# rfahd1525/Block-Blast-AI---Reinforcement-Learning-Agent

Measured on NVIDIA B200. Metric: env_steps_per_sec, higher is better.
Workload: dtype u64

## Files before the change

block-blast-ai---reinforcement-learning-agent_b200/csrc/bb_env_kernels.cu:

```cuda
#include <cuda_runtime.h>
#include "bb_rules.cuh"
#include "bb_kernels.h"

__device__ BBTables g_bb_tables = {BB_PIECE_ROWS};

__device__ __forceinline__ void bb_load_state(const BBEnvArrays& E, int64_t i, BBState& s) {
    const uint4 a = E.s0[i], b = E.s1[i], c = E.s2[i];
    s.board = (uint64_t)a.x | ((uint64_t)a.y << 32);
    s.pieces = a.z;
    s.aux = a.w;
    s.score = (int32_t)b.x; s.streak = (int32_t)b.y; s.moves = (int32_t)b.z; s.lines_total = (int32_t)b.w;
    s.max_streak = (int32_t)c.x; s.blocks_total = (int32_t)c.y; s.draw_ctr = c.z; s.policy_ctr = c.w;
}

__device__ __forceinline__ void bb_store_state(const BBEnvArrays& E, int64_t i, const BBState& s) {
    E.s0[i] = make_uint4((uint32_t)s.board, (uint32_t)(s.board >> 32), s.pieces, s.aux);
    E.s1[i] = make_uint4((uint32_t)s.score, (uint32_t)s.streak, (uint32_t)s.moves, (uint32_t)s.lines_total);
    E.s2[i] = make_uint4((uint32_t)s.max_streak, (uint32_t)s.blocks_total, s.draw_ctr, s.policy_ctr);
}

__device__ __forceinline__ uint64_t bb_shfl64(uint64_t v, int src) {
    const uint32_t lo = __shfl_sync(0xffffffffu, (uint32_t)v, src);
    const uint32_t hi = __shfl_sync(0xffffffffu, (uint32_t)(v >> 32), src);
    return (uint64_t)lo | ((uint64_t)hi << 32);
}

#ifdef BB_PROFILE
struct BBProf { long long cls = 0, team = 0, rounds = 0, iters = 0, t0 = 0, c0 = 0, c1 = 0, q0 = 0, q1 = 0, units = 0, units_all = 0, unit_cyc = 0; };
__device__ unsigned long long g_pf_units = 0, g_pf_units_max = 0, g_pf_open_cyc = 0, g_pf_unit_cyc = 0, g_pf_H = 0;
#define BB_PF(...) __VA_ARGS__
#else
struct BBProf {};
#define BB_PF(...)
#endif

__device__ __forceinline__ bool bb_warp_solve(bool hard, const BBItem& item, uint32_t trio, const BBTables* T,
                                              BBProf& pf) {
    const unsigned FULL = 0xffffffffu;
    const int lane = threadIdx.x & 31;
    bool solved = false;
    uint32_t next = 0;
    const uint32_t nbr = BB_PLAN_NA(item.plan) + BB_PLAN_NB(item.plan);
    unsigned hmask = __ballot_sync(FULL, hard);
    while (hmask) {
        BB_PF(pf.rounds += 1;)
        const int rem = hard ? (int)(nbr - next) : 0;
        int excl = 32;
        int owner = lane, o_excl = 0, o_rem = 0;
        bool in_team = false;
        int run = 0;
        for (unsigned m = hmask; m && run < 32; m &= m - 1u) {
            const int h = __ffs((int)m) - 1;
            const int r = __shfl_sync(FULL, rem, h);
            if (lane == h) excl = run;
            if (lane >= run && lane < run + r) { owner = h; o_excl = run; o_rem = r; in_team = true; }
            run += r;
        }
        const int served_o = min(o_rem, 32 - o_excl);
        const unsigned team_mask = in_team ? ((served_o >= 32 ? FULL : ((1u << served_o) - 1u)) << o_excl) : 0u;
        BBItem it;
        it.b = bb_shfl64(item.b, owner);
        it.v[0] = bb_shfl64(item.v[0], owner);
        it.v[1] = bb_shfl64(item.v[1], owner);
        it.v[2] = bb_shfl64(item.v[2], owner);
        it.plan = __shfl_sync(FULL, item.plan, owner);
        const uint32_t tr = __shfl_sync(FULL, trio, owner);
        const uint32_t t = __shfl_sync(FULL, next, owner) + (uint32_t)(lane - o_excl);
        BBBranch br;
        br.bb = 0; br.m0 = 0; br.m1 = 0; br.always = 0;
        br.A.pm = br.A.inb = br.A.offs = 0; br.A.meta = 0;
        br.B = br.A;
        BB_PF(pf.q0 = clock64();)
        if (in_team) bb_branch_open(br, it, T, tr, t);
        BB_PF(pf.q1 = clock64(); pf.units = 0;)
        unsigned found = 0;
        for (;;) {
            const bool work = in_team && !(found & team_mask) && ((br.m0 | br.m1) != 0ull);
            if (!__any_sync(FULL, work)) break;
            bool f = false;
            if (work) f = bb_branch_unit(br);
            found |= __ballot_sync(FULL, f);
            BB_PF(pf.units += 1;)
        }
        BB_PF(if (lane == 0) {
            pf.units_all += pf.units; pf.unit_cyc += clock64() - pf.q1;
            atomicAdd(&g_pf_units, (unsigned long long)pf.units);
            atomicMax(&g_pf_units_max, (unsigned long long)pf.units);
            atomicAdd(&g_pf_open_cyc, (unsigned long long)(pf.q1 - pf.q0));
            atomicAdd(&g_pf_unit_cyc, (unsigned long long)(clock64() - pf.q1));
            atomicAdd(&g_pf_H, (unsigned long long)__popc(hmask));
        })
        if (hard) {
            const int served = max(0, min(rem, 32 - excl));
            const unsigned tm = served > 0 ? ((served >= 32 ? FULL : ((1u << served) - 1u)) << excl) : 0u;
            next += (uint32_t)served;
            if (found & tm) { hard = false; solved = true; }
            else if (next >= nbr) hard = false;
        }
        hmask = __ballot_sync(FULL, hard);
    }
    return solved;
}

template <class Src>
__device__ __forceinline__ uint32_t bb_warp_deal(bool pending, uint64_t board, const BBTables* T,
                                                 const Src& src, uint64_t env_id, uint32_t& pieces,
                                                 uint32_t& draw_ctr, BBProf& pf) {
    const unsigned FULL = 0xffffffffu;
    const int lane = threadIdx.x & 31;
    uint32_t attempts = 0;
    unsigned pmask = __ballot_sync(FULL, pending);
    while (pmask) {
        BB_PF(pf.c0 = clock64(); pf.iters += 1;)
        const int P = __popc(pmask);
        const int w = 32 / P;
        const int g = lane / w, r = lane - g * w;
        const bool in_grp = g < P;
        const int owner = in_grp ? bb_select((uint64_t)pmask, g) : lane;
        const unsigned grp_bits = (w == 32 ? FULL : ((1u << w) - 1u));
        const int shift = (in_grp ? g : 0) * w;
        const uint64_t ob = bb_shfl64(board, owner);
        const uint64_t oid = bb_shfl64(env_id, owner);
        const uint32_t octr = __shfl_sync(FULL, draw_ctr, owner);
        const uint32_t oatt = __shfl_sync(FULL, attempts, owner);
        const bool cand = in_grp && (oatt + (uint32_t)r < 100u);
        BBItem item;
        item.b = ob; item.v[0] = item.v[1] = item.v[2] = 0; item.plan = 0;
        uint32_t trio = 0;
        int cls = BB_REJECT;
        if (cand) {
            trio = bb_candidate(src, oid, octr + (uint32_t)r);
            cls = bb_classify(ob, bb_piece(T, trio & 0xFFu), bb_piece(T, (trio >> 8) & 0xFFu),
                              bb_piece(T, (trio >> 16) & 0xFFu), &item);
        }
        const unsigned amask = __ballot_sync(FULL, cls == BB_ACCEPT);
        const unsigned ga = (amask >> shift) & grp_bits;
        const int first_acc = ga ? (__ffs((int)ga) - 1) : w;
        const bool hard = cand && cls == BB_HARD && r < first_acc;
        BB_PF(pf.c1 = clock64(); pf.cls += pf.c1 - pf.c0;)
        const bool solved = bb_warp_solve(hard, item, trio, T, pf);
        BB_PF(pf.team += clock64() - pf.c1;)
        const unsigned okmask = __ballot_sync(FULL, cand && (cls == BB_ACCEPT || solved));
        const unsigned go = (okmask >> shift) & grp_bits;
        const int nvalid = (int)min((uint32_t)w, 100u - oatt);
        const int take = go ? __ffs((int)go) : nvalid;
        const bool done = go != 0u || (oatt + (uint32_t)take >= 100u);
        const uint32_t chosen = __shfl_sync(FULL, trio, (in_grp ? g * w : 0) + take - 1);
        const int my_base = pending ? __popc(pmask & ((1u << lane) - 1u)) * w : 0;
        const int t_take = __shfl_sync(FULL, take, my_base);
        const int t_done = __shfl_sync(FULL, (int)done, my_base);
        const uint32_t t_trio = __shfl_sync(FULL, chosen, my_base);
        if (pending) {
            draw_ctr += (uint32_t)t_take;
            attempts += (uint32_t)t_take;
            pieces = t_trio;
            pending = !t_done;
        }
        pmask = __ballot_sync(FULL, pending);
    }
    return attempts;
}

template <bool RANDOM, bool INJECT>
__global__ void __launch_bounds__(BB_STEP_THREADS, BB_STEP_MIN_BLOCKS)
bb_step_kernel(BBEnvArrays E, BBRewardCfg cfg, const int32_t* __restrict__ actions, int n_steps, int per_step,
               int32_t* __restrict__ actions_out, float* __restrict__ rewards,
               uint8_t* __restrict__ terminated, uint64_t* __restrict__ mask_out,
               int32_t* __restrict__ ep_score, int32_t* __restrict__ ep_len,
               uint32_t* __restrict__ info_out, unsigned long long* __restrict__ stats,
               uint64_t* __restrict__ board_out, uint32_t* __restrict__ pieces_out,
               const uint64_t* __restrict__ mask_in) {
    const BBTables& T = g_bb_tables;
    const int64_t i = (int64_t)blockIdx.x * blockDim.x + threadIdx.x;
    const bool live = i < E.n;
    unsigned st_eps = 0, st_score = 0, st_len = 0, st_max = 0;
    BBTrioSrc src(E.seed);
    if (INJECT) { src.trios = E.trios; src.len = E.trio_len; src.base = E.trio_base; }
    BBState s;
    BBStepOut o;
    int action = 0;
    const uint64_t env_id = (uint64_t)(E.env_offset + (live ? i : 0));
    if (live) {
        bb_load_state(E, i, s);
        if (RANDOM) {
            if (mask_in) {
                const int64_t ms = E.out_stride ? E.out_stride : E.n;
                o.mask[0] = mask_in[i]; o.mask[1] = mask_in[ms + i]; o.mask[2] = mask_in[2 * ms + i];
            } else {
                bb_action_mask(s, &T, o.mask);
            }
        } else {
            action = actions[i];
        }
    } else {
        s.board = 0; s.pieces = 0; s.aux = 0; s.draw_ctr = 0; s.policy_ctr = 0;
        s.score = s.streak = s.moves = s.lines_total = s.max_streak = s.blocks_total = 0;
        o.mask[0] = o.mask[1] = o.mask[2] = 0;
    }
    const int steps = RANDOM ? n_steps : 1;
    BBProf pf;
    BB_PF(pf.t0 = clock64();)
    for (int step = 0; step < steps; ++step) {
        BBMove mv;
        mv.ok = false; mv.needs_deal = false; mv.n = 0; mv.lines = 0; mv.gain = 0;
        if (live) {
            if (RANDOM) {
                const BBPhilox4 r = bb_philox((uint32_t)env_id, (uint32_t)(env_id >> 32), s.policy_ctr,
                                              BB_STREAM_POLICY, (uint32_t)E.seed, (uint32_t)(E.seed >> 32));
                s.policy_ctr += 1;
                action = bb_pick_action(o.mask, r.x);
            }
            mv = bb_env_pre(s, action, &T, o);
        }
        const uint32_t draws = bb_warp_deal(live && mv.ok && mv.needs_deal, s.board, &T, src, env_id,
                                            s.pieces, s.draw_ctr, pf);
        if (live && mv.ok) {
            bb_env_post(s, mv, draws, &T, cfg, src, env_id, E.flags, o, E.ep_end ? E.ep_end + i : nullptr);
            if (o.terminated) {
                st_eps += 1u; st_score += (unsigned)o.ep_score; st_len += (unsigned)o.ep_len;
                st_max = max(st_max, (unsigned)o.ep_score);
            }
        }
        if (RANDOM && per_step && live) {
            const int64_t base = (int64_t)step * E.n + i;
            if (actions_out) actions_out[base] = action;
            if (rewards) rewards[base] = o.reward;
            if (terminated) terminated[base] = (uint8_t)o.terminated;
            if (mask_out) {
                const int64_t mb = (int64_t)step * 3 * E.n + i;
                mask_out[mb] = o.mask[0];
                mask_out[mb + E.n] = o.mask[1];
                mask_out[mb + 2 * E.n] = o.mask[2];
            }
        }
    }
    if (RANDOM && per_step) {
        if (live) bb_store_state(E, i, s);
        actions_out = nullptr; rewards = nullptr; terminated = nullptr; mask_out = nullptr;
    }
    if (live) {
        if (!(RANDOM && per_step)) bb_store_state(E, i, s);
        if (RANDOM && actions_out) actions_out[i] = action;
        if (rewards) rewards[i] = o.reward;
        if (terminated) terminated[i] = (uint8_t)o.terminated;
        if (mask_out) {
            const int64_t ms = E.out_stride ? E.out_stride : E.n;
            mask_out[i] = o.mask[0];
            mask_out[ms + i] = o.mask[1];
            mask_out[2 * ms + i] = o.mask[2];
        }
        if (o.terminated) {
            if (ep_score) ep_score[i] = o.ep_score;
            if (ep_len) ep_len[i] = o.ep_len;
        }
        if (info_out) info_out[i] = o.info;
        if (board_out) board_out[i] = s.board;
        if (pieces_out) pieces_out[i] = s.pieces;
    }
    if (stats) {
        const unsigned FULLM = 0xffffffffu;
        const unsigned long long w_eps = __reduce_add_sync(FULLM, st_eps);
        const unsigned long long w_score = (unsigned long long)__reduce_add_sync(FULLM, st_score & 0xFFFFu) +
                                           ((unsigned long long)__reduce_add_sync(FULLM, st_score >> 16) << 16);
        const unsigned long long w_len = (unsigned long long)__reduce_add_sync(FULLM, st_len & 0xFFFFu) +
                                         ((unsigned long long)__reduce_add_sync(FULLM, st_len >> 16) << 16);
        const unsigned w_max = __reduce_max_sync(FULLM, st_max);
        const unsigned long long nlive = __popc(__ballot_sync(0xffffffffu, live));
        if ((threadIdx.x & 31) == 0) {
            BB_PF(const unsigned long long tot = (unsigned long long)(clock64() - pf.t0);
                  atomicAdd(&stats[4], tot);
                  atomicAdd(&stats[5], (unsigned long long)pf.cls);
                  atomicAdd(&stats[6], (unsigned long long)pf.team);
                  atomicAdd(&stats[7], (unsigned long long)pf.rounds);
                  atomicAdd(&stats[8], (unsigned long long)pf.iters);
                  atomicMax(&stats[9], tot);
                  atomicMax(&stats[10], (unsigned long long)pf.rounds);
                  atomicMax(&stats[63 - (tot & 7)], (tot << 32) | (((unsigned long long)pf.unit_cyc >> 6) << 16) |
                                                        ((unsigned long long)(pf.units_all > 255 ? 255 : pf.units_all) << 8) | (unsigned long long)(pf.rounds > 255 ? 255 : pf.rounds));
                  stats[11] = g_pf_units; stats[12] = g_pf_units_max; stats[13] = g_pf_open_cyc;
                  stats[14] = g_pf_unit_cyc; stats[15] = g_pf_H;
                  atomicAdd(&stats[16 + (tot >> 13 > 31 ? 31 : tot >> 13)], 1ull);
                  atomicAdd(&stats[48 + (pf.rounds > 7 ? 7 : pf.rounds)], 1ull);)
            atomicAdd(&stats[0], nlive * (unsigned long long)n_steps);
            if (w_eps) {
                atomicAdd(&stats[1], w_eps);
                atomicAdd(&stats[2], w_score);
                atomicAdd(&stats[3], w_len);
#ifndef BB_PROFILE
                atomicMax(&stats[4], (unsigned long long)w_max);
#endif
            }
        }
    }
}

__global__ void __launch_bounds__(BB_STEP_THREADS)
bb_reset_kernel(BBEnvArrays E, const uint8_t* __restrict__ reset_mask, uint64_t* __restrict__ mask_out) {
    const BBTables& T = g_bb_tables;
    const int64_t i = (int64_t)blockIdx.x * blockDim.x + threadIdx.x;
    if (i >= E.n) return;
    BBState s;
    bb_load_state(E, i, s);
    if (!reset_mask || reset_mask[i]) {
        BBTrioSrc src(E.seed);
        src.trios = E.trios; src.len = E.trio_len; src.base = E.trio_base;
        bb_reset_state(s, src, (uint64_t)(E.env_offset + i), E.flags);
        bb_store_state(E, i, s);
    }
    if (mask_out) {
        uint64_t m[3];
        bb_action_mask(s, &T, m);
        mask_out[i] = m[0];
        mask_out[E.n + i] = m[1];
        mask_out[2 * E.n + i] = m[2];
    }
}

__global__ void __launch_bounds__(BB_STEP_THREADS)
bb_observe_kernel(BBEnvArrays E, uint64_t* __restrict__ board_out, uint32_t* __restrict__ pieces_out,
                  uint64_t* __restrict__ mask_out) {
    const BBTables& T = g_bb_tables;
    const int64_t i = (int64_t)blockIdx.x * blockDim.x + threadIdx.x;
    if (i >= E.n) return;
    BBState s;
    bb_load_state(E, i, s);
    if (board_out) board_out[i] = s.board;
    if (pieces_out) pieces_out[i] = s.pieces;
    if (mask_out) {
        uint64_t m[3];
        bb_action_mask(s, &T, m);
        mask_out[i] = m[0];
        mask_out[E.n + i] = m[1];
        mask_out[2 * E.n + i] = m[2];
    }
}

#define BB_STREAM_SAMPLE_VALID 3u
__global__ void __launch_bounds__(BB_STEP_THREADS)
bb_sample_valid_kernel(BBEnvArrays E, uint64_t call_counter, int32_t* __restrict__ actions_out) {
    const BBTables& T = g_bb_tables;
    const int64_t i = (int64_t)blockIdx.x * blockDim.x + threadIdx.x;
    if (i >= E.n) return;
    BBState s;
    bb_load_state(E, i, s);
    uint64_t m[3];
    bb_action_mask(s, &T, m);
    const uint64_t env_id = (uint64_t)(E.env_offset + i);
    const BBPhilox4 r = bb_philox((uint32_t)env_id, (uint32_t)(env_id >> 32), (uint32_t)call_counter,
                                  BB_STREAM_SAMPLE_VALID, (uint32_t)E.seed, (uint32_t)(E.seed >> 32));
    actions_out[i] = bb_pick_action(m, r.x);
}

__device__ __forceinline__ int64_t bb_warp_incl_scan(int64_t v) {
    const int lane = threadIdx.x & 31;
#pragma unroll
    for (int o = 1; o < 32; o <<= 1) {
        const int64_t u = __shfl_up_sync(0xffffffffu, v, o);
        if (lane >= o) v += u;
    }
    return v;
}

__device__ __forceinline__ int64_t bb_block_incl_scan(int64_t v, int64_t* total) {
    __shared__ int64_t warp_sums[BB_STEP_THREADS / 32];
    const int lane = threadIdx.x & 31, w = threadIdx.x >> 5;
    v = bb_warp_incl_scan(v);
    if (lane == 31) warp_sums[w] = v;
    __syncthreads();
    if (w == 0) {
        int64_t t = lane < BB_STEP_THREADS / 32 ? warp_sums[lane] : 0;
        t = bb_warp_incl_scan(t);
        if (lane < BB_STEP_THREADS / 32) warp_sums[lane] = t;
    }
// ... 194 lines not shown
```

block-blast-ai---reinforcement-learning-agent_b200/csrc/bb_rules.cuh:

```cuda
#pragma once
#include <stdint.h>

#if defined(__CUDACC__)
#define BB_HD __host__ __device__ __forceinline__
#else
#define BB_HD inline
#endif

#include "bb_piece_table.inc"

#define BB_TABLE_N (BB_NUM_PIECES + 3)
struct alignas(16) BBTableRow {
    uint64_t mask;
    uint64_t inb;
    uint64_t offs;
    uint32_t meta;
    uint32_t pad;
};
struct BBTables { BBTableRow row[BB_TABLE_N]; };

#define BB_META_N(m) ((m) & 0xFu)
#define BB_META_MAXROW(m) (((m) >> 12) & 0xFu)
#define BB_META_MAXCOL(m) (((m) >> 16) & 0xFu)

static const uint64_t BB_HOST_PIECE_MASKS[BB_NUM_PIECES] = BB_PIECE_MASKS;
static const uint64_t BB_HOST_PIECE_INB[BB_NUM_PIECES] = BB_PIECE_INB;
static const uint64_t BB_HOST_PIECE_OFFS[BB_NUM_PIECES] = BB_PIECE_OFFS;
static const uint32_t BB_HOST_PIECE_META[BB_NUM_PIECES] = BB_PIECE_META;

inline void bb_fill_tables(BBTables* t) {
    for (int i = 0; i < BB_TABLE_N; ++i) {
        t->row[i].mask = i < BB_NUM_PIECES ? BB_HOST_PIECE_MASKS[i] : 0;
        t->row[i].inb = i < BB_NUM_PIECES ? BB_HOST_PIECE_INB[i] : 0;
        t->row[i].offs = i < BB_NUM_PIECES ? BB_HOST_PIECE_OFFS[i] : 0;
        t->row[i].meta = i < BB_NUM_PIECES ? BB_HOST_PIECE_META[i] : 0;
        t->row[i].pad = 0;
    }
}

struct BBPiece { uint64_t pm, inb, offs; uint32_t meta; };

BB_HD BBPiece bb_piece(const BBTables* T, uint32_t id) {
    BBPiece p;
#if defined(__CUDA_ARCH__)
    const uint4* r = reinterpret_cast<const uint4*>(&T->row[id]);
    const uint4 a = r[0], b = r[1];
    p.pm = (uint64_t)a.x | ((uint64_t)a.y << 32);
    p.inb = (uint64_t)a.z | ((uint64_t)a.w << 32);
    p.offs = (uint64_t)b.x | ((uint64_t)b.y << 32);
    p.meta = b.z;
#else
    p.pm = T->row[id].mask; p.inb = T->row[id].inb; p.offs = T->row[id].offs; p.meta = T->row[id].meta;
#endif
    return p;
}

BB_HD int bb_popc(uint64_t x) {
#if defined(__CUDA_ARCH__)
    return __popcll(x);
#else
    return __builtin_popcountll(x);
#endif
}
BB_HD int bb_popc32(uint32_t x) {
#if defined(__CUDA_ARCH__)
    return __popc(x);
#else
    return __builtin_popcount(x);
#endif
}
BB_HD int bb_ctz(uint64_t x) {
#if defined(__CUDA_ARCH__)
    const uint32_t lo = (uint32_t)x;
    return lo ? (__ffs((int)lo) - 1) : (31 + __ffs((int)(uint32_t)(x >> 32)));
#else
    return __builtin_ctzll(x);
#endif
}
BB_HD uint32_t bb_mulhi(uint32_t a, uint32_t b) {
#if defined(__CUDA_ARCH__)
    return __umulhi(a, b);
#else
    return (uint32_t)(((uint64_t)a * b) >> 32);
#endif
}
BB_HD int bb_select(uint64_t w, int k) {
#if defined(__CUDA_ARCH__)
    uint32_t x = (uint32_t)w;
    int pos = 0;
    int c = __popc(x);
    if (k >= c) { k -= c; pos = 32; x = (uint32_t)(w >> 32); }
    c = __popc(x & 0xFFFFu);
    if (k >= c) { k -= c; pos += 16; x >>= 16; }
    c = __popc(x & 0xFFu);
    if (k >= c) { k -= c; pos += 8; x >>= 8; }
    c = __popc(x & 0xFu);
    if (k >= c) { k -= c; pos += 4; x >>= 4; }
    c = __popc(x & 0x3u);
    if (k >= c) { k -= c; pos += 2; x >>= 2; }
    if (k >= (int)(x & 1u)) pos += 1;
    return pos;
#else
    for (int i = 0; i < k; ++i) w &= w - 1;
    return __builtin_ctzll(w);
#endif
}

#define BB_COL_A 0x0101010101010101ull
#define BB_COL_H 0x8080808080808080ull
#define BB_CENTER 0x00003C3C3C3C0000ull

BB_HD uint64_t bb_shr(uint64_t e, uint32_t o) {
#if defined(__CUDA_ARCH__)
    const uint32_t lo = (uint32_t)e, hi = (uint32_t)(e >> 32);
    return (uint64_t)__funnelshift_rc(lo, hi, o) | ((uint64_t)__funnelshift_rc(hi, 0u, o) << 32);
#else
    return e >> o;
#endif
}

BB_HD uint32_t bb_byte(uint32_t w, int k) {
#if defined(__CUDA_ARCH__)
    return __byte_perm(w, 0u, 0x4440u + (uint32_t)k);
#else
    return (w >> (8 * k)) & 0xFFu;
#endif
}

BB_HD uint64_t bb_valid(uint64_t e, const BBPiece& p) {
    const uint32_t lo = (uint32_t)p.offs, hi = (uint32_t)(p.offs >> 32);
    uint64_t v = bb_shr(e, bb_byte(lo, 0)) & bb_shr(e, bb_byte(lo, 1));
    v &= bb_shr(e, bb_byte(lo, 2)) & bb_shr(e, lo >> 24);
    v &= bb_shr(v, bb_byte(hi, 0));
    v &= bb_shr(v, bb_byte(hi, 1));
    return v & p.inb;
}

BB_HD uint32_t bb_rowflags32(uint32_t x) { return ((x & 0x7F7F7F7Fu) + 0x01010101u) & x; }
BB_HD uint32_t bb_rowmask32(uint32_t x) {
#if defined(__CUDA_ARCH__)
    uint32_t m;
    asm("prmt.b32 %0, %1, %2, %3;" : "=r"(m) : "r"(bb_rowflags32(x)), "r"(0u), "r"(0xBA98u));
    return m;
#else
    return ((bb_rowflags32(x) & 0x80808080u) >> 7) * 0xFFu;
#endif
}
BB_HD uint32_t bb_fullcols(uint32_t lo, uint32_t hi) {
    uint32_t c = lo & hi;
    c &= c >> 16;
    c &= c >> 8;
    return c & 0xFFu;
}

BB_HD uint64_t bb_clear(uint64_t b, int* lines) {
    const uint32_t lo = (uint32_t)b, hi = (uint32_t)(b >> 32);
    const uint32_t rl = bb_rowmask32(lo), rh = bb_rowmask32(hi), c = bb_fullcols(lo, hi);
    const uint32_t cm = c * 0x01010101u;
    *lines = ((bb_popc32(rl) + bb_popc32(rh)) >> 3) + bb_popc32(c);
    return (uint64_t)(lo & ~(rl | cm)) | ((uint64_t)(hi & ~(rh | cm)) << 32);
}

BB_HD bool bb_any_full(uint64_t b) {
    const uint32_t lo = (uint32_t)b, hi = (uint32_t)(b >> 32);
    return ((((bb_rowflags32(lo) | bb_rowflags32(hi)) & 0x80808080u) | bb_fullcols(lo, hi))) != 0u;
}

BB_HD uint64_t bb_clear_only(uint64_t b) {
    int l;
    return bb_clear(b, &l);
}

BB_HD uint64_t bb_clear_if_full(uint64_t b, bool* full) {
    const uint32_t lo = (uint32_t)b, hi = (uint32_t)(b >> 32);
    const uint32_t rl = bb_rowmask32(lo), rh = bb_rowmask32(hi), c = bb_fullcols(lo, hi);
    const uint32_t cm = c * 0x01010101u;
    *full = (rl | rh | c) != 0u;
    return (uint64_t)(lo & ~(rl | cm)) | ((uint64_t)(hi & ~(rh | cm)) << 32);
}

BB_HD int bb_holes(uint64_t b) {
    const uint64_t up = (b << 8) | 0xFFull;
    const uint64_t dn = (b >> 8) | 0xFF00000000000000ull;
    const uint64_t lf = ((b << 1) & ~BB_COL_A) | BB_COL_A;
    const uint64_t rt = ((b >> 1) & ~BB_COL_H) | BB_COL_H;
    return bb_popc(~b & up & dn & lf & rt);
}

BB_HD int bb_center(uint64_t b) { return bb_popc(b & BB_CENTER); }

struct BBLines { uint64_t rows; uint32_t colp; };

BB_HD uint32_t bb_maj(uint32_t x, uint32_t y, uint32_t z) { return (x & y) | (x & z) | (y & z); }

BB_HD BBLines bb_lines(uint64_t b) {
    BBLines L;
    uint64_t t = b - ((b >> 1) & 0x5555555555555555ull);
    t = (t & 0x3333333333333333ull) + ((t >> 2) & 0x3333333333333333ull);
    L.rows = (t + (t >> 4)) & 0x0F0F0F0F0F0F0F0Full;
    const uint32_t lo = (uint32_t)b, hi = (uint32_t)(b >> 32);
    const uint32_t a1 = lo ^ hi, b1 = lo & hi;
    const uint32_t c = a1 & (a1 >> 16);
    const uint32_t a2 = a1 ^ (a1 >> 16), b2 = b1 ^ (b1 >> 16) ^ c, d2 = bb_maj(b1, b1 >> 16, c);
    const uint32_t c1 = a2 & (a2 >> 8);
    const uint32_t ones = a2 ^ (a2 >> 8), twos = b2 ^ (b2 >> 8) ^ c1, c2 = bb_maj(b2, b2 >> 8, c1);
    const uint32_t fours = d2 ^ (d2 >> 8) ^ c2, eights = bb_maj(d2, d2 >> 8, c2);
    L.colp = (ones & 0xFFu) | ((twos & 0xFFu) << 8) | ((fours & 0xFFu) << 16) | ((eights & 0xFFu) << 24);
    return L;
}
BB_HD uint64_t bb_rows_within_mask(const BBLines& L, int m) {
    const uint64_t f = L.rows + (uint64_t)(0x78 + m) * BB_COL_A;
#if defined(__CUDA_ARCH__)
    uint32_t lo, hi;
    asm("prmt.b32 %0, %1, %2, %3;" : "=r"(lo) : "r"((uint32_t)f), "r"(0u), "r"(0xBA98u));
    asm("prmt.b32 %0, %1, %2, %3;" : "=r"(hi) : "r"((uint32_t)(f >> 32)), "r"(0u), "r"(0xBA98u));
    return (uint64_t)lo | ((uint64_t)hi << 32);
#else
    return ((f & BB_COL_H) >> 7) * 0xFFull;
#endif
}
BB_HD uint32_t bb_cols_within_bits(const BBLines& L, int m) {
    const uint32_t ones = L.colp & 0xFFu, twos = (L.colp >> 8) & 0xFFu, fours = (L.colp >> 16) & 0xFFu, eights = L.colp >> 24;
    const uint32_t m0 = 0u - ((uint32_t)m & 1u), m1 = 0u - (((uint32_t)m >> 1) & 1u), m2 = 0u - (((uint32_t)m >> 2) & 1u);
    const uint32_t k0 = ones & m0;
    const uint32_t k1 = bb_maj(twos, m1, k0);
    const uint32_t k2 = bb_maj(fours, m2, k1);
    return (eights | k2) & 0xFFu;
}
BB_HD bool bb_row_within(const BBLines& L, int m) {
    return ((L.rows + (uint64_t)(0x78 + m) * BB_COL_A) & BB_COL_H) != 0;
}
BB_HD bool bb_col_within(const BBLines& L, int m) { return bb_cols_within_bits(L, m) != 0u; }

BB_HD uint64_t bb_cover(uint64_t T, const BBPiece& p) {
    const uint32_t lo = (uint32_t)p.offs, hi = (uint32_t)(p.offs >> 32);
    uint64_t v = bb_shr(T, bb_byte(lo, 0)) | bb_shr(T, bb_byte(lo, 1));
    v |= bb_shr(T, bb_byte(lo, 2)) | bb_shr(T, lo >> 24);
    v |= bb_shr(v, bb_byte(hi, 0));
    v |= bb_shr(v, bb_byte(hi, 1));
    return v;
}

BB_HD uint64_t bb_clearing_candidates(uint64_t bb, const BBLines& L, const BBPiece& p) {
    const uint64_t near = bb_rows_within_mask(L, (int)BB_META_MAXROW(p.meta)) |
                          ((uint64_t)bb_cols_within_bits(L, (int)BB_META_MAXCOL(p.meta)) * BB_COL_A);
    return bb_cover(~bb & near, p);
}

struct BBPhilox4 { uint32_t x, y, z, w; };

BB_HD BBPhilox4 bb_philox(uint32_t c0, uint32_t c1, uint32_t c2, uint32_t c3, uint32_t k0, uint32_t k1) {
#pragma unroll
    for (int i = 0; i < 10; ++i) {
        const uint32_t hi0 = bb_mulhi(0xD2511F53u, c0), lo0 = 0xD2511F53u * c0;
        const uint32_t hi1 = bb_mulhi(0xCD9E8D57u, c2), lo1 = 0xCD9E8D57u * c2;
        c0 = hi1 ^ c1 ^ k0;
        c1 = lo1;
        c2 = hi0 ^ c3 ^ k1;
        c3 = lo0;
        k0 += 0x9E3779B9u;
        k1 += 0xBB67AE85u;
    }
    BBPhilox4 r = {c0, c1, c2, c3};
    return r;
}

#define BB_STREAM_TRIO 0u
#define BB_STREAM_POLICY 1u
#define BB_STREAM_SAMPLE 2u

BB_HD uint32_t bb_draw_trio(uint64_t seed, uint64_t env_id, uint32_t draw) {
    const BBPhilox4 r = bb_philox((uint32_t)env_id, (uint32_t)(env_id >> 32), draw, BB_STREAM_TRIO,
                                  (uint32_t)seed, (uint32_t)(seed >> 32));
    return bb_mulhi(r.x, 37u) | (bb_mulhi(r.y, 37u) << 8) | (bb_mulhi(r.z, 37u) << 16);
}

struct BBTrioSrc {
    uint64_t seed;
    const uint8_t* trios;
    int64_t len, base;
    BB_HD BBTrioSrc(uint64_t s = 0) : seed(s), trios(nullptr), len(0), base(0) {}
};

BB_HD uint32_t bb_candidate(const BBTrioSrc& src, uint64_t env_id, uint32_t draw) {
    if (src.trios) {
        const uint8_t* t = src.trios + (((int64_t)env_id - src.base) * src.len + (int64_t)(draw % (uint32_t)src.len)) * 3;
        return (uint32_t)t[0] | ((uint32_t)t[1] << 8) | ((uint32_t)t[2] << 16);
    }
    return bb_draw_trio(src.seed, env_id, draw);
}

#define BB_STREAM_LOOKAHEAD 4u
struct BBLookaheadSrc {
    uint64_t seed;
    uint32_t call_counter;
};

BB_HD uint32_t bb_candidate(const BBLookaheadSrc& src, uint64_t env_id, uint32_t draw) {
    const BBPhilox4 r = bb_philox((uint32_t)env_id, (uint32_t)(env_id >> 32), (src.call_counter << 7) | (draw & 0xFFu),
                                  BB_STREAM_LOOKAHEAD | (draw >> 8 << 8), (uint32_t)src.seed, (uint32_t)(src.seed >> 32));
    return bb_mulhi(r.x, 37u) | (bb_mulhi(r.y, 37u) << 8) | (bb_mulhi(r.z, 37u) << 16);
}

#ifdef BB_COUNT_WORK
struct BBWork { long long valid_calls, fast_accept, fast_reject, pack_iters, clear_iters, slow, branches; };
static BBWork g_bb_work;
#define BB_WORK(f, n) (g_bb_work.f += (n))
#else
#define BB_WORK(f, n) ((void)0)
#endif

enum { BB_REJECT = 0, BB_ACCEPT = 1, BB_HARD = 2 };

struct BBItem {
    uint64_t b;
    uint64_t v[3];
    uint32_t plan;
};
#define BB_PLAN_NA(p) (((p) >> 8) & 0xFFu)
#define BB_PLAN_NB(p) (((p) >> 16) & 0xFFu)

BB_HD BBPiece bb_pick3(const BBPiece& p0, const BBPiece& p1, const BBPiece& p2, int i) {
    BBPiece r;
    r.pm = i == 0 ? p0.pm : (i == 1 ? p1.pm : p2.pm);
    r.inb = i == 0 ? p0.inb : (i == 1 ? p1.inb : p2.inb);
    r.offs = i == 0 ? p0.offs : (i == 1 ? p1.offs : p2.offs);
    r.meta = i == 0 ? p0.meta : (i == 1 ? p1.meta : p2.meta);
    return r;
}

BB_HD bool bb_clear_reachable(uint64_t b, const BBPiece& p0, const BBPiece& p1, const BBPiece& p2) {
    const int r0 = (int)BB_META_MAXROW(p0.meta), r1 = (int)BB_META_MAXROW(p1.meta), r2 = (int)BB_META_MAXROW(p2.meta);
    const int c0 = (int)BB_META_MAXCOL(p0.meta), c1 = (int)BB_META_MAXCOL(p1.meta), c2 = (int)BB_META_MAXCOL(p2.meta);
    const int rmin = r0 < r1 ? (r0 < r2 ? r0 : r2) : (r1 < r2 ? r1 : r2);
    const int cmin = c0 < c1 ? (c0 < c2 ? c0 : c2) : (c1 < c2 ? c1 : c2);
    const int rt = r0 + r1 + r2 - rmin, ct = c0 + c1 + c2 - cmin;
    if (rt >= 8 || ct >= 8) return true;
    const BBLines L = bb_lines(b);
    return bb_row_within(L, rt) || bb_col_within(L, ct);
}

BB_HD int bb_classify(uint64_t b, const BBPiece& p0, const BBPiece& p1, const BBPiece& p2, BBItem* it) {
    const uint64_t e = ~b;
    it->b = b;
    it->v[0] = bb_valid(e, p0);
    it->v[1] = bb_valid(e, p1);
    it->v[2] = bb_valid(e, p2);
    BB_WORK(valid_calls, 3);
    const int n0 = bb_popc(it->v[0]), n1 = bb_popc(it->v[1]), n2 = bb_popc(it->v[2]);
    uint32_t nA = 0, order = 0;
    if (n0 && n1 && n2) {
        int x = 0, y = 1, z = 2;
        if (n1 < n0 && n1 <= n2) { x = 1; y = 0; }
        else if (n2 < n0 && n2 < n1) { x = 2; z = 0; }
        const int ny = (y == 0 ? n0 : (y == 1 ? n1 : n2)), nz = (z == 0 ? n0 : (z == 1 ? n1 : n2));
        if (nz < ny) { const int s_ = y; y = z; z = s_; }
        const BBPiece px = bb_pick3(p0, p1, p2, x), py = bb_pick3(p0, p1, p2, y), pz = bb_pick3(p0, p1, p2, z);
        const uint64_t vx = x == 0 ? it->v[0] : (x == 1 ? it->v[1] : it->v[2]);
        const uint64_t b1 = b | (px.pm << bb_ctz(vx));
        const uint64_t vy = bb_valid(~b1, py);
        BB_WORK(valid_calls, 1);
        if (vy) {
            BB_WORK(valid_calls, 1);
            if (bb_valid(~(b1 | (py.pm << bb_ctz(vy))), pz)) return BB_ACCEPT;
            const int ah = 63 - (int)
#if defined(__CUDA_ARCH__)
                __clzll((long long)vy);
#else
                __builtin_clzll(vy);
#endif
            BB_WORK(valid_calls, 1);
            if (bb_valid(~(b1 | (py.pm << ah)), pz)) return BB_ACCEPT;
        }
        nA = (uint32_t)(x == 0 ? n0 : (x == 1 ? n1 : n2));
        order = (uint32_t)x | ((uint32_t)y << 2) | ((uint32_t)z << 4);
    }
    const uint32_t nB = bb_clear_reachable(b, p0, p1, p2) ? (uint32_t)(n0 + n1 + n2) : 0u;
    it->plan = order | (nA << 8) | (nB << 16);
    if (nA + nB == 0) return BB_REJECT;
    return BB_HARD;
}

struct BBBranch {
    uint64_t bb, m0, m1;
    BBPiece A, B;
    uint32_t always;
};

BB_HD bool bb_can_complete_line(const BBLines& L, const BBPiece& p) {
    return bb_row_within(L, (int)BB_META_MAXROW(p.meta)) || bb_col_within(L, (int)BB_META_MAXCOL(p.meta));
}

#define BB_TRIO_ID(trio, i) (((trio) >> (8 * (i))) & 0xFFu)

BB_HD uint64_t bb_one_anchor_if_roomy(uint64_t mA, uint64_t vB, const BBPiece& A, const BBPiece& B) {
    const int roomy = bb_popc(vB) > (int)(BB_META_N(A.meta) * BB_META_N(B.meta));
    return roomy ? (mA & (0ull - mA)) : mA;
}

BB_HD void bb_branch_open(BBBranch& br, const BBItem& it, const BBTables* T, uint32_t trio, uint32_t t) {
    BB_WORK(branches, 1);
    const uint32_t nA = BB_PLAN_NA(it.plan);
    if (t < nA) {
        const int x = (int)(it.plan & 3u), y = (int)((it.plan >> 2) & 3u), z = (int)((it.plan >> 4) & 3u);
        const uint64_t vx = x == 0 ? it.v[0] : (x == 1 ? it.v[1] : it.v[2]);
        const uint64_t pmx = T->row[BB_TRIO_ID(trio, x)].mask;
        bool full;
        br.bb = bb_clear_if_full(it.b | (pmx << bb_select(vx, (int)t)), &full);
        br.A = bb_piece(T, BB_TRIO_ID(trio, y));
        br.B = bb_piece(T, BB_TRIO_ID(trio, z));
        BB_WORK(valid_calls, 2);
        const uint64_t vA = bb_valid(~br.bb, br.A), vB = bb_valid(~br.bb, br.B);
        const bool flip = bb_popc(vB) < bb_popc(vA);
        const uint64_t vf = flip ? vB : vA, vs = flip ? vA : vB;
        br.m0 = vs ? bb_one_anchor_if_roomy(vf, vs, br.A, br.B) : 0ull;
        br.m1 = 0ull;
        br.always = 1u | (flip ? 4u : 0u);
        return;
    }
    int k = (int)(t - nA);
    int i = 0;
    const int n0 = bb_popc(it.v[0]), n1 = bb_popc(it.v[1]);
    if (k >= n0) { k -= n0; i = 1; if (k >= n1) { k -= n1; i = 2; } }
    const int j = i == 0 ? 1 : 0, l = i == 2 ? 1 : 2;
    const uint64_t vi = i == 0 ? it.v[0] : (i == 1 ? it.v[1] : it.v[2]);
    const uint64_t pmi = T->row[BB_TRIO_ID(trio, i)].mask;
    bool full1;
    br.bb = bb_clear_if_full(it.b | (pmi << bb_select(vi, k)), &full1);
    br.A = bb_piece(T, BB_TRIO_ID(trio, j));
    br.B = bb_piece(T, BB_TRIO_ID(trio, l));
    const BBLines L = bb_lines(br.bb);
    BB_WORK(valid_calls, 2);
    const uint64_t vA = bb_valid(~br.bb, br.A), vB = bb_valid(~br.bb, br.B);
    const uint64_t cA = vA & bb_clearing_candidates(br.bb, L, br.A), cB = vB & bb_clearing_candidates(br.bb, L, br.B);
    const bool flip = full1 && bb_popc(vB) < bb_popc(vA);
    br.m0 = full1 ? bb_one_anchor_if_roomy(flip ? vB : vA, flip ? vA : vB, br.A, br.B) : cA;
    br.m1 = flip ? cA : cB;
    br.always = (full1 ? 1u : 0u) | (flip ? 4u : 0u);
}

BB_HD bool bb_branch_unit(BBBranch& br) {
    const bool ph = br.m0 == 0ull;
    uint64_t m = ph ? br.m1 : br.m0;
    const int a = bb_ctz(m);
    m &= m - 1;
    if (ph) br.m1 = m; else br.m0 = m;
    const bool useB = ph != (((br.always >> 2) & 1u) != 0u);
    bool full;
    const uint64_t b2 = bb_clear_if_full(br.bb | ((useB ? br.B.pm : br.A.pm) << a), &full);
    BB_WORK(clear_iters, 1);
    if (!full && !((br.always >> (ph ? 1 : 0)) & 1u)) return false;
    BB_WORK(valid_calls, 1);
    BBPiece s2;
    s2.pm = 0;
    s2.inb = useB ? br.A.inb : br.B.inb;
    s2.offs = useB ? br.A.offs : br.B.offs;
    s2.meta = useB ? br.A.meta : br.B.meta;
    return bb_valid(~b2, s2) != 0ull;
}

BB_HD bool bb_branch(const BBItem& it, const BBTables* T, uint32_t trio, uint32_t t) {
    BBBranch br;
    bb_branch_open(br, it, T, trio, t);
    while (br.m0 | br.m1)
        if (bb_branch_unit(br)) return true;
    return false;
}

BB_HD bool bb_solvable(uint64_t b, const BBTables* T, uint32_t trio) {
    BBPiece P[3];
    P[0] = bb_piece(T, trio & 0xFFu);
    P[1] = bb_piece(T, (trio >> 8) & 0xFFu);
    P[2] = bb_piece(T, (trio >> 16) & 0xFFu);
    BBItem it;
    const int f = bb_classify(b, P[0], P[1], P[2], &it);
    if (f == BB_ACCEPT) { BB_WORK(fast_accept, 1); return true; }
    if (f == BB_REJECT) { BB_WORK(fast_reject, 1); return false; }
    BB_WORK(slow, 1);
    const uint32_t n = BB_PLAN_NA(it.plan) + BB_PLAN_NB(it.plan);
    for (uint32_t t = 0; t < n; ++t)
        if (bb_branch(it, T, trio, t)) return true;
    return false;
}

struct BBState {
    uint64_t board;
    uint32_t pieces;
    uint32_t aux;
    int32_t score, streak, moves, lines_total;
    int32_t max_streak, blocks_total;
    uint32_t draw_ctr;
    uint32_t policy_ctr;
};

#define BB_USED(s) (((s).pieces >> 24) & 7u)
#define BB_OVER(s) (((s).aux >> 16) & 1u)

struct BBRewardCfg {
    double line_clear_base, block_placed, game_over_penalty, hole_penalty, center_bonus,
        combo_multiplier_bonus, survival_bonus;
};

#define BB_FLAG_RESEED_ON_RESET 1u
#define BB_FLAG_NO_AUTO_RESET 2u

BB_HD double bb_dmul(double a, double b) {
#if defined(__CUDA_ARCH__)
    return __dmul_rn(a, b);
#else
    volatile double r = a * b; return r;
#endif
}
BB_HD double bb_dadd(double a, double b) {
#if defined(__CUDA_ARCH__)
    return __dadd_rn(a, b);
#else
    volatile double r = a + b; return r;
#endif
}

BB_HD float bb_reward(const BBRewardCfg& c, int n_blocks, int lines, bool game_over,
                      int holes, int prev_holes, int center, int prev_center) {
    double r = bb_dadd(0.0, bb_dmul((double)n_blocks, c.block_placed));
    r = bb_dadd(r, c.survival_bonus);
    if (lines > 0) {
        const int cmul = lines < 4 ? lines : 4;
        double lr = bb_dmul((double)lines, c.line_clear_base);
        lr = bb_dmul(lr, (double)cmul);
        r = bb_dadd(r, lr);
        if (cmul > 1) r = bb_dadd(r, bb_dmul((double)(cmul - 1), c.combo_multiplier_bonus));
    }
    if (game_over) r = bb_dadd(r, c.game_over_penalty);
    const int d = holes - prev_holes;
    if (d > 0) r = bb_dadd(r, bb_dmul((double)d, c.hole_penalty));
    if (center <= prev_center) r = bb_dadd(r, bb_dmul(c.center_bonus, 0.1));
    return (float)r;
}

template <class Src>
BB_HD uint32_t bb_deal(uint64_t board, const BBTables* T, const Src& src, uint64_t env_id, uint32_t* draw_ctr) {
    uint32_t trio = 0;
    for (int attempt = 0; attempt < 100; ++attempt) {
        trio = bb_candidate(src, env_id, *draw_ctr);
        *draw_ctr += 1;
        if (bb_solvable(board, T, trio)) break;
    }
    return trio;
}

BB_HD void bb_reset_state(BBState& s, const BBTrioSrc& src, uint64_t env_id, uint32_t flags) {
    if (flags & BB_FLAG_RESEED_ON_RESET) s.draw_ctr = 0;
    s.board = 0;
    s.score = s.streak = s.moves = s.lines_total = s.max_streak = s.blocks_total = 0;
    s.aux = 0;
    s.pieces = bb_candidate(src, env_id, s.draw_ctr);
    s.draw_ctr += 1;
}

BB_HD void bb_action_mask(const BBState& s, const BBTables* T, uint64_t m[3]) {
    const uint64_t e = ~s.board;
    const uint32_t used = BB_USED(s);
    const bool over = BB_OVER(s);
#pragma unroll
    for (int i = 0; i < 3; ++i) {
        const uint64_t v = bb_valid(e, bb_piece(T, (s.pieces >> (8 * i)) & 0xFFu));
        m[i] = (((used >> i) & 1u) || over) ? 0ull : v;
    }
}

struct BBStepOut {
    float reward;
    uint32_t terminated;
    uint32_t info;
    int32_t gain;
    int32_t ep_score, ep_len;
    uint64_t mask[3];
};

struct BBMove { int n, lines, gain; bool ok, needs_deal; };

struct BBEpisodeEnd {
    uint64_t board;
    uint32_t pieces;
    int32_t lines_total, max_streak, blocks_total;
    uint32_t holes_fill;
    uint32_t last_move;
};

BB_HD BBMove bb_env_pre(BBState& s, int action, const BBTables* T, BBStepOut& o) {
    BBMove mv;
    mv.n = 0; mv.lines = 0; mv.gain = 0; mv.needs_deal = false;
    const uint32_t used = BB_USED(s);
    const int p = action >> 6;
    const int a = action & 63;
    bool ok = (action >= 0) && (p < 3) && !((used >> (p & 3)) & 1u) && !BB_OVER(s);
    const uint32_t id = ok ? ((s.pieces >> (8 * p)) & 0xFFu) : 0u;
    const uint64_t pm = T->row[id].mask;
    if (ok) ok = ((T->row[id].inb >> a) & 1ull) && (((pm << a) & s.board) == 0ull);
    mv.ok = ok;
    o.ep_score = 0; o.ep_len = 0; o.gain = 0;
    if (!ok) {
        o.reward = -10.0f;
        o.terminated = 0;
        o.info = 1u;
        bb_action_mask(s, T, o.mask);
        return mv;
    }
    const int n = (int)BB_META_N(T->row[id].meta);
    int lines;
    s.board = bb_clear(s.board | (pm << a), &lines);
    const uint32_t used2 = used | (1u << p);
    s.moves += 1;
    s.blocks_total += n;
    int gain = n;
    if (lines > 0) {
        s.streak += 1;
        s.max_streak = s.max_streak > s.streak ? s.max_streak : s.streak;
        s.lines_total += lines;
        const int cmul = lines < 4 ? lines : 4;
        const int smul = s.streak + 1 < 8 ? s.streak + 1 : 8;
        gain += lines * 80 * cmul * smul;
    } else {
        s.streak = 0;
    }
    s.score += gain;
    s.pieces = (s.pieces & 0x00FFFFFFu) | (used2 << 24);
    mv.n = n; mv.lines = lines; mv.gain = gain;
    mv.needs_deal = used2 == 7u;
    return mv;
}

BB_HD void bb_env_post(BBState& s, const BBMove& mv, uint32_t draws, const BBTables* T, const BBRewardCfg& cfg,
                       const BBTrioSrc& src, uint64_t env_id, uint32_t flags, BBStepOut& o, BBEpisodeEnd* ep_end = nullptr) {
    bb_action_mask(s, T, o.mask);
    const bool over = (o.mask[0] | o.mask[1] | o.mask[2]) == 0ull;
    const int h = bb_holes(s.board), ctr = bb_center(s.board);
    o.reward = bb_reward(cfg, mv.n, mv.lines, over, h, (int)(s.aux & 0xFFu), ctr, (int)((s.aux >> 8) & 0xFFu));
    s.aux = (uint32_t)h | ((uint32_t)ctr << 8) | ((over ? 1u : 0u) << 16);
    o.terminated = over ? 1u : 0u;
    o.gain = mv.gain;
    o.info = ((uint32_t)mv.lines << 1) | ((uint32_t)mv.n << 4) |
             ((uint32_t)(mv.lines > 0 ? (mv.lines < 4 ? mv.lines : 4) : 1) << 8) | (draws << 11) |
             ((uint32_t)mv.gain << 18);
    if (over) {
        o.ep_score = s.score;
        o.ep_len = s.moves;
        if (ep_end) {
            ep_end->board = s.board; ep_end->pieces = s.pieces;
            ep_end->lines_total = s.lines_total; ep_end->max_streak = s.max_streak; ep_end->blocks_total = s.blocks_total;
            ep_end->holes_fill = (uint32_t)h | ((uint32_t)bb_popc(s.board) << 8);
            ep_end->last_move = o.info;
        }
        if (!(flags & BB_FLAG_NO_AUTO_RESET)) {
            bb_reset_state(s, src, env_id, flags);
            o.mask[0] = T->row[s.pieces & 0xFFu].inb;
            o.mask[1] = T->row[(s.pieces >> 8) & 0xFFu].inb;
            o.mask[2] = T->row[(s.pieces >> 16) & 0xFFu].inb;
        }
    }
}

BB_HD void bb_env_apply(BBState& s, int action, const BBTables* T, const BBRewardCfg& cfg,
                        const BBTrioSrc& src, uint64_t env_id, uint32_t flags, BBStepOut& o) {
    const BBMove mv = bb_env_pre(s, action, T, o);
    if (!mv.ok) return;
    uint32_t draws = 0;
    if (mv.needs_deal) {
        const uint32_t before = s.draw_ctr;
        s.pieces = bb_deal(s.board, T, src, env_id, &s.draw_ctr);
        draws = s.draw_ctr - before;
    }
    bb_env_post(s, mv, draws, T, cfg, src, env_id, flags, o);
}

BB_HD int bb_kth_action(const uint64_t m[3], int k) {
    const int n0 = bb_popc(m[0]), n1 = bb_popc(m[1]);
    int p = 0;
    uint64_t w = m[0];
    if (k >= n0) { k -= n0; p = 1; w = m[1]; if (k >= n1) { k -= n1; p = 2; w = m[2]; } }
    return p * 64 + bb_select(w, k);
}

BB_HD int bb_pick_action(const uint64_t m[3], uint32_t word) {
    const int total = bb_popc(m[0]) + bb_popc(m[1]) + bb_popc(m[2]);
    if (total == 0) return 0;
    return bb_kth_action(m, (int)bb_mulhi(word, (uint32_t)total));
}

BB_HD bool bb_expand_deals(const BBState& s) { return bb_popc32(BB_USED(s)) == 2; }

BB_HD int bb_expand_count(const BBState& s, const uint64_t m[3], int samples) {
    const int n = bb_popc(m[0]) + bb_popc(m[1]) + bb_popc(m[2]);
    return bb_expand_deals(s) ? n * samples : n;
}

BB_HD int bb_expand_item(const BBState& s, const uint64_t m[3], int samples, int j, int* k) {
    int a = j;
    *k = 0;
    if (bb_expand_deals(s)) { a = j / samples; *k = j - a * samples; }
    return bb_kth_action(m, a);
}
```

Before: 6.512 billion.

## Replace variable shifts in piece placement masks with multiplies and table pointers

bb_valid and bb_cover now compute the shifted board masks as 32x64 multiplies by precomputed powers of two, with one final right shift, in place of six variable 64-bit funnel shifts with byte extraction. The piece table is rebuilt at compile time with per-piece multipliers and a top shift. A static_assert checks that every piece's offsets fit the multiply form. BBPiece now carries a pointer to its table row, and the multiplier fields are loaded through __ldg on use. This cuts register pressure from carrying inb and offs in BBPiece, at the cost of extra memory loads per valid or cover call.

```diff
diff --git a/block-blast-ai---reinforcement-learning-agent_b200/csrc/bb_env_kernels.cu b/block-blast-ai---reinforcement-learning-agent_b200/csrc/bb_env_kernels.cu
--- a/block-blast-ai---reinforcement-learning-agent_b200/csrc/bb_env_kernels.cu
+++ b/block-blast-ai---reinforcement-learning-agent_b200/csrc/bb_env_kernels.cu
@@ -2,7 +2,7 @@
 #include "bb_rules.cuh"
 #include "bb_kernels.h"
 
-__device__ BBTables g_bb_tables = {BB_PIECE_ROWS};
+__device__ BBTables g_bb_tables = bb_make_tables();
 
 __device__ __forceinline__ void bb_load_state(const BBEnvArrays& E, int64_t i, BBState& s) {
     const uint4 a = E.s0[i], b = E.s1[i], c = E.s2[i];
@@ -68,7 +68,7 @@
         const uint32_t t = __shfl_sync(FULL, next, owner) + (uint32_t)(lane - o_excl);
         BBBranch br;
         br.bb = 0; br.m0 = 0; br.m1 = 0; br.always = 0;
-        br.A.pm = br.A.inb = br.A.offs = 0; br.A.meta = 0;
+        br.A.pm = 0; br.A.row = T->row; br.A.meta = 0;
         br.B = br.A;
         BB_PF(pf.q0 = clock64();)
         if (in_team) bb_branch_open(br, it, T, tr, t);
diff --git a/block-blast-ai---reinforcement-learning-agent_b200/csrc/bb_rules.cuh b/block-blast-ai---reinforcement-learning-agent_b200/csrc/bb_rules.cuh
--- a/block-blast-ai---reinforcement-learning-agent_b200/csrc/bb_rules.cuh
+++ b/block-blast-ai---reinforcement-learning-agent_b200/csrc/bb_rules.cuh
@@ -13,9 +13,10 @@
 struct alignas(16) BBTableRow {
     uint64_t mask;
     uint64_t inb;
-    uint64_t offs;
+    uint32_t mul[4];
+    uint32_t mb1, mb2;
     uint32_t meta;
-    uint32_t pad;
+    uint32_t top;
 };
 struct BBTables { BBTableRow row[BB_TABLE_N]; };
 
@@ -23,35 +24,55 @@
 #define BB_META_MAXROW(m) (((m) >> 12) & 0xFu)
 #define BB_META_MAXCOL(m) (((m) >> 16) & 0xFu)
 
-static const uint64_t BB_HOST_PIECE_MASKS[BB_NUM_PIECES] = BB_PIECE_MASKS;
-static const uint64_t BB_HOST_PIECE_INB[BB_NUM_PIECES] = BB_PIECE_INB;
-static const uint64_t BB_HOST_PIECE_OFFS[BB_NUM_PIECES] = BB_PIECE_OFFS;
-static const uint32_t BB_HOST_PIECE_META[BB_NUM_PIECES] = BB_PIECE_META;
-
-inline void bb_fill_tables(BBTables* t) {
-    for (int i = 0; i < BB_TABLE_N; ++i) {
-        t->row[i].mask = i < BB_NUM_PIECES ? BB_HOST_PIECE_MASKS[i] : 0;
-        t->row[i].inb = i < BB_NUM_PIECES ? BB_HOST_PIECE_INB[i] : 0;
-        t->row[i].offs = i < BB_NUM_PIECES ? BB_HOST_PIECE_OFFS[i] : 0;
-        t->row[i].meta = i < BB_NUM_PIECES ? BB_HOST_PIECE_META[i] : 0;
-        t->row[i].pad = 0;
-    }
-}
-
-struct BBPiece { uint64_t pm, inb, offs; uint32_t meta; };
+static constexpr uint64_t BB_HOST_PIECE_MASKS[BB_NUM_PIECES] = BB_PIECE_MASKS;
+static constexpr uint64_t BB_HOST_PIECE_INB[BB_NUM_PIECES] = BB_PIECE_INB;
+static constexpr uint64_t BB_HOST_PIECE_OFFS[BB_NUM_PIECES] = BB_PIECE_OFFS;
+static constexpr uint32_t BB_HOST_PIECE_META[BB_NUM_PIECES] = BB_PIECE_META;
+
+constexpr uint32_t bb_offs_byte(int piece, int k) { return (uint32_t)(BB_HOST_PIECE_OFFS[piece] >> (8 * k)) & 0xFFu; }
+constexpr uint32_t bb_offs_base_max(int piece) {
+    uint32_t o = 0;
+    for (int k = 0; k < 4; ++k) o = bb_offs_byte(piece, k) > o ? bb_offs_byte(piece, k) : o;
+    return o;
+}
+constexpr uint32_t bb_offs_top(int piece) { return bb_offs_base_max(piece) + bb_offs_byte(piece, 4) + bb_offs_byte(piece, 5); }
+
+constexpr BBTables bb_make_tables() {
+    BBTables t{};
+    for (int i = 0; i < BB_NUM_PIECES; ++i) {
+        BBTableRow& r = t.row[i];
+        r.mask = BB_HOST_PIECE_MASKS[i];
+        r.inb = BB_HOST_PIECE_INB[i];
+        for (int k = 0; k < 4; ++k) r.mul[k] = 1u << (bb_offs_base_max(i) - bb_offs_byte(i, k));
+        r.mb1 = 1u << bb_offs_byte(i, 4);
+        r.mb2 = 1u << bb_offs_byte(i, 5);
+        r.meta = BB_HOST_PIECE_META[i];
+        r.top = bb_offs_top(i);
+    }
+    return t;
+}
+
+constexpr bool bb_recipe_in_range() {
+    for (int i = 0; i < BB_NUM_PIECES; ++i) {
+        for (int k = 0; k < 6; ++k)
+            if (bb_offs_byte(i, k) > 31u) return false;
+        if (bb_offs_top(i) > 32u) return false;
+        if ((BB_HOST_PIECE_MASKS[i] >> bb_offs_top(i)) != 1ull) return false;
+    }
+    return true;
+}
+static_assert(bb_recipe_in_range(), "piece recipe outside the range of bb_valid's multiply form");
+
+inline void bb_fill_tables(BBTables* t) { *t = bb_make_tables(); }
+
+struct BBPiece { uint64_t pm; const BBTableRow* row; uint32_t meta; };
 
 BB_HD BBPiece bb_piece(const BBTables* T, uint32_t id) {
     BBPiece p;
-#if defined(__CUDA_ARCH__)
-    const uint4* r = reinterpret_cast<const uint4*>(&T->row[id]);
-    const uint4 a = r[0], b = r[1];
-    p.pm = (uint64_t)a.x | ((uint64_t)a.y << 32);
-    p.inb = (uint64_t)a.z | ((uint64_t)a.w << 32);
-    p.offs = (uint64_t)b.x | ((uint64_t)b.y << 32);
-    p.meta = b.z;
-#else
-    p.pm = T->row[id].mask; p.inb = T->row[id].inb; p.offs = T->row[id].offs; p.meta = T->row[id].meta;
-#endif
+    const BBTableRow* r = &T->row[id];
+    p.pm = r->mask;
+    p.row = r;
+    p.meta = r->meta;
     return p;
 }
 
@@ -119,21 +140,38 @@
 #endif
 }
 
-BB_HD uint32_t bb_byte(uint32_t w, int k) {
-#if defined(__CUDA_ARCH__)
-    return __byte_perm(w, 0u, 0x4440u + (uint32_t)k);
-#else
-    return (w >> (8 * k)) & 0xFFu;
-#endif
+BB_HD uint64_t bb_mulshl(uint64_t e, uint32_t m) {
+#if defined(__CUDA_ARCH__)
+    uint64_t w;
+    asm("mul.wide.u32 %0, %1, %2;" : "=l"(w) : "r"((uint32_t)e), "r"(m));
+#else
+    const uint64_t w = (uint64_t)(uint32_t)e * m;
+#endif
+    const uint32_t hi = (uint32_t)(e >> 32) * m + (uint32_t)(w >> 32);
+    return (w & 0xFFFFFFFFull) | ((uint64_t)hi << 32);
+}
+
+struct BBMuls { uint32_t a0, a1, a2, a3, b1, b2, t; uint64_t inb; };
+
+BB_HD BBMuls bb_muls(const BBTableRow* r) {
+    BBMuls k;
+#if defined(__CUDA_ARCH__)
+    const uint4 a = __ldg(reinterpret_cast<const uint4*>(r->mul));
+    const uint4 b = __ldg(reinterpret_cast<const uint4*>(&r->mb1));
+    k.a0 = a.x; k.a1 = a.y; k.a2 = a.z; k.a3 = a.w; k.b1 = b.x; k.b2 = b.y; k.t = b.w;
+    k.inb = __ldg(reinterpret_cast<const unsigned long long*>(&r->inb));
+#else
+    k.a0 = r->mul[0]; k.a1 = r->mul[1]; k.a2 = r->mul[2]; k.a3 = r->mul[3]; k.b1 = r->mb1; k.b2 = r->mb2; k.t = r->top; k.inb = r->inb;
+#endif
+    return k;
 }
 
 BB_HD uint64_t bb_valid(uint64_t e, const BBPiece& p) {
-    const uint32_t lo = (uint32_t)p.offs, hi = (uint32_t)(p.offs >> 32);
-    uint64_t v = bb_shr(e, bb_byte(lo, 0)) & bb_shr(e, bb_byte(lo, 1));
-    v &= bb_shr(e, bb_byte(lo, 2)) & bb_shr(e, lo >> 24);
-    v &= bb_shr(v, bb_byte(hi, 0));
-    v &= bb_shr(v, bb_byte(hi, 1));
-    return v & p.inb;
+    const BBMuls k = bb_muls(p.row);
+    uint64_t v = bb_mulshl(e, k.a0) & bb_mulshl(e, k.a1) & bb_mulshl(e, k.a2) & bb_mulshl(e, k.a3);
+    v &= bb_mulshl(v, k.b1);
+    v &= bb_mulshl(v, k.b2);
+    return bb_shr(v, k.t) & k.inb;
 }
 
 BB_HD uint32_t bb_rowflags32(uint32_t x) { return ((x & 0x7F7F7F7Fu) + 0x01010101u) & x; }
@@ -233,12 +271,11 @@
 BB_HD bool bb_col_within(const BBLines& L, int m) { return bb_cols_within_bits(L, m) != 0u; }
 
 BB_HD uint64_t bb_cover(uint64_t T, const BBPiece& p) {
-    const uint32_t lo = (uint32_t)p.offs, hi = (uint32_t)(p.offs >> 32);
-    uint64_t v = bb_shr(T, bb_byte(lo, 0)) | bb_shr(T, bb_byte(lo, 1));
-    v |= bb_shr(T, bb_byte(lo, 2)) | bb_shr(T, lo >> 24);
-    v |= bb_shr(v, bb_byte(hi, 0));
-    v |= bb_shr(v, bb_byte(hi, 1));
-    return v;
+    const BBMuls k = bb_muls(p.row);
+    uint64_t v = bb_mulshl(T, k.a0) | bb_mulshl(T, k.a1) | bb_mulshl(T, k.a2) | bb_mulshl(T, k.a3);
+    v |= bb_mulshl(v, k.b1);
+    v |= bb_mulshl(v, k.b2);
+    return bb_shr(v, k.t);
 }
 
 BB_HD uint64_t bb_clearing_candidates(uint64_t bb, const BBLines& L, const BBPiece& p) {
@@ -323,8 +360,7 @@
 BB_HD BBPiece bb_pick3(const BBPiece& p0, const BBPiece& p1, const BBPiece& p2, int i) {
     BBPiece r;
     r.pm = i == 0 ? p0.pm : (i == 1 ? p1.pm : p2.pm);
-    r.inb = i == 0 ? p0.inb : (i == 1 ? p1.inb : p2.inb);
-    r.offs = i == 0 ? p0.offs : (i == 1 ? p1.offs : p2.offs);
+    r.row = i == 0 ? p0.row : (i == 1 ? p1.row : p2.row);
     r.meta = i == 0 ? p0.meta : (i == 1 ? p1.meta : p2.meta);
     return r;
 }
@@ -453,8 +489,7 @@
     BB_WORK(valid_calls, 1);
     BBPiece s2;
     s2.pm = 0;
-    s2.inb = useB ? br.A.inb : br.B.inb;
-    s2.offs = useB ? br.A.offs : br.B.offs;
+    s2.row = useB ? br.A.row : br.B.row;
     s2.meta = useB ? br.A.meta : br.B.meta;
     return bb_valid(~b2, s2) != 0ull;
 }
```

New measurement: 6.223 billion (median of 6 runs). 4.4% lower.
